# mathwrx/Decouple-and-Couple_Learning_in_Multi-Modal_Brain_Tumor_Segmentation

Hardware: AMD Instinct MI355X
Metric: training volumes/sec (4x128^3) (higher is better)
Workload: dtype bf16x3 forward (split-bf16 MFMA operands hi.hi+hi.lo+lo.hi: logits within 1e-3 of the fp32 reference) / bf16 data-gradient / bf16 weight-gradient MFMA operands; f32 accumulate, f32 storage, f32 master weights; 1 GPU; configs[1]: 1xMI355X, batch 2 per GPU, 4-modality 128^3 synthetic BraTS patches; fwd + softmax_dice + 4 sub-region/edge losses + bwd + Adam(amsgrad); random-init weights, dropout on; global_batch=2, parallelism=dp1, precision=bf16x3, dgrad_precision=bf16, wgrad_precision=bf16, mode=plan

## Files before the change

### decouple-and-couple_learning_in_multi-modal_brain_tumor_segmentation_amd/csrc/conv_args.h

```cpp
#pragma once
#include "common.h"

typedef __bf16 bf16x8 __attribute__((ext_vector_type(8)));
typedef unsigned u32x4 __attribute__((ext_vector_type(4)));

struct ConvArgsB {
  ConvGeom g;
  const float* x; const uint4* wpk; const float* bias; float* y;
  const float* in_scale; const float* in_shift; float in_slope;
  const float* residual; int r_ldc; const float* out_scale; double* stats;
  unsigned long long unused_[2];
  const float* nb_x; int nb_ldc; const float* nb_scale; const float* nb_shift; float nb_slope;
  int groups, x_goff, y_goff;
  const uint4* wpk_g[3]; const float* bias_g[3];
  const uint4* x16; const uint4* zero16;
  unsigned short* y16;
};

typedef __bf16 bf16x2_t __attribute__((ext_vector_type(2)));
typedef float f32x2_t __attribute__((ext_vector_type(2)));
__device__ __forceinline__ unsigned pack_bf16(float a, float b) {
  const f32x2_t f = {a, b};
  return __builtin_bit_cast(unsigned, __builtin_convertvector(f, bf16x2_t));
}
__device__ __forceinline__ float bf16_round(float a) { return (float)(__bf16)a; }
__device__ __forceinline__ void split_bf16(float a, float b, unsigned& hi, unsigned& lo) {
  hi = pack_bf16(a, b);
  const float ha = __builtin_bit_cast(float, hi << 16), hb = __builtin_bit_cast(float, hi & 0xffff0000u);
  lo = pack_bf16(a - ha, b - hb);
}
__device__ __forceinline__ float act01(float v, float slope) { return fmaxf(v, v * slope); }


static inline int cfg_extent(int op, int Di, int Hi, int Wi, int Do, int Ho, int Wo, int cd[3]) {
  cd[0] = Do; cd[1] = Ho; cd[2] = Wo;
  if (op == CWF_CONVT2) { cd[0] = Di; cd[1] = Hi; cd[2] = Wi; return 8; }
  if (op == CWF_CONV3_S2_DGRAD) { cd[0] = (Do + 1) / 2; cd[1] = (Ho + 1) / 2; cd[2] = (Wo + 1) / 2; return 8; }
  return 1;
}

int cwf_try_conv_ws(int op, int x3, ConvArgsB& a, hipStream_t st, int* rc);
int cwf_ws_takes_x16(int op, int N, int D, int H, int W, int Cin, int Cout);
int cwf_ws_takes_x3();
int cwf_try_conv_wsp(int op, int x3, int cfg_mt, int cfg_wm, ConvArgsB& a, hipStream_t st, int* rc);
int cwf_try_conv_wsd(int op, int x3, int cfg_mt, int cfg_wm, ConvArgsB& a, hipStream_t st, int* rc);

int conv_fp32_launch(const cwf_conv_args& d, hipStream_t st);
int conv_stem_launch(const cwf_conv_args& d, hipStream_t st);
int conv_s2c16_launch(const cwf_conv_args& d, hipStream_t st);
int wgrad_fp32_launch(const cwf_wgrad_args& d, int* nsplit_used, hipStream_t st);
```

### decouple-and-couple_learning_in_multi-modal_brain_tumor_segmentation_amd/csrc/conv_bf16.hip

```cpp
#include "common.h"
#include <cstdio>
#include <cstdlib>
#include <type_traits>

#include "conv_args.h"

#define CB_MAXS 13
struct StageSlots { int goff[CB_MAXS]; unsigned inb; int nslots; };

__device__ __forceinline__ void stage_slots_init(StageSlots& ss, const ConvGeom& g, int id0, int ih0, int iw0, int tid) {
  const int nvox_in = g.ID * g.IH * g.IW;
  ss.nslots = (nvox_in + 63) >> 6; ss.inb = 0u;
  const int dq = 64 / g.IW, dr = 64 - dq * g.IW;
  int iw = (tid >> 2) % g.IW, t2 = (tid >> 2) / g.IW;
  int ih = t2 % g.IH, idd = t2 / g.IH;
#pragma unroll
  for (int i = 0; i < CB_MAXS; ++i) {
    const int v = (tid >> 2) + 64 * i;
    const int gd = id0 + idd, gh = ih0 + ih, gw = iw0 + iw;
    const bool ok = v < nvox_in && gd >= 0 && gd < g.Di && gh >= 0 && gh < g.Hi && gw >= 0 && gw < g.Wi;
    ss.goff[i] = ok ? ((gd * g.Hi + gh) * g.Wi + gw) * g.x_ldc : 0;
    ss.inb |= ok ? (1u << i) : 0u;
    iw += dr; int adv = dq;
    if (iw >= g.IW) { iw -= g.IW; ++adv; }
// ... 1072 lines not shown
    const double reuse = 1.0 - 0.35 / (c.MT * c.NT) - 0.1 / MTOT;
    const double score = sp_eff * n_eff * fill * reuse;
    if (score > best_score) { best_score = score; best = c; }
  }
  return best;
}

template <int MT, int NT, int WM, bool X3>
int launch_cfg(const ConvArgsB& a, hipStream_t st) {
  constexpr int WN = 4 / WM;
  const ConvGeom& g = a.g;
  const size_t lds_tile = (size_t)g.ID * g.IH * g.IW * 16 * sizeof(unsigned short) * (X3 ? 2 : 1);
  const size_t lds_red = (size_t)4 * NT * 16 * 2 * sizeof(float);
  const size_t lds = lds_tile > lds_red ? lds_tile : lds_red;
  if (lds > 160 * 1024) return CWF_E_TOOLARGE;
  CWF_MAX_LDS_ONCE((&conv_bf16_kernel<MT, NT, WM, X3>));
  dim3 grid(g.tiles_d * g.tiles_h * g.tiles_w, cdiv(g.ntiles, WN * NT), g.N * g.ncls * (a.groups ? a.groups : 1));
  hipLaunchKernelGGL((conv_bf16_kernel<MT, NT, WM, X3>), grid, dim3(256), lds, st, a);
  CWF_LAUNCH_CHECK();
  return 0;
}
}

extern "C" int cwf_debug_conv_bf16_cfg(int op, int N, int Di, int Hi, int Wi, int Do, int Ho, int Wo, int Cout, int* mt_nt_wm) {
  if (!mt_nt_wm || N <= 0 || Di <= 0 || Hi <= 0 || Wi <= 0 || Do <= 0 || Ho <= 0 || Wo <= 0 || Cout <= 0 || op < CWF_CONV3_S1 ||
      op > CWF_CONVT2_DGRAD)
    return CWF_E_BADARG;
  int cd[3];
  const int ncls = cfg_extent(op, Di, Hi, Wi, Do, Ho, Wo, cd);
  const TileCfg c = choose_cfg(op, cd, ncls, N, cdiv(Cout, 16));
  mt_nt_wm[0] = c.MT; mt_nt_wm[1] = c.NT; mt_nt_wm[2] = c.WM;
  return 0;
}

static void c16_tap_order(ConvGeom& g) {
  int nat[27];
  for (int t = 0; t < 27; ++t) nat[t] = g.tapofs[t];
  for (int t = 0; t < 27; ++t) g.tapofs[t] = nat[c16_tap(t)];
}

static int conv_bf16_impl(const cwf_conv_args& d, hipStream_t st) {
  const int op = d.op, x3 = d.precision == CWF_BF16X3, N = d.N, Cin = d.Cin, Cout = d.Cout, y_ldc = d.y_ldc;
  const float* x = d.x16 ? reinterpret_cast<const float*>(d.x16) : d.x;
  const int x_ldc = d.x16 ? Cin : d.x_ldc;
  if (!x || !d.wpk || !d.y || N <= 0 || Cin <= 0 || Cout <= 0) return CWF_E_BADARG;
  if (d.nb_x && (!d.stats || !d.nb_scale || !d.nb_shift || d.nb_ldc < Cout)) return CWF_E_BADARG;
  if ((Cin & 3) || (x_ldc & 3) || x_ldc < Cin || y_ldc < Cout) return CWF_E_ALIGN;
  if (((uintptr_t)x & 15) || ((uintptr_t)d.wpk & 15)) return CWF_E_ALIGN;
  if (d.in_scale && !d.in_shift) return CWF_E_BADARG;
  ConvArgsB a;
  int cd[3];
  const int ncls = cfg_extent(op, d.Di, d.Hi, d.Wi, d.Do, d.Ho, d.Wo, cd);
  const TileCfg c = choose_cfg(op, cd, ncls, N, cdiv(Cout, 16));
  int rc = cwf_build_geom(a.g, op, N, d.Di, d.Hi, d.Wi, Cin, x_ldc, d.Do, d.Ho, d.Wo, Cout, y_ldc, c.MT * c.WM);
  if (rc) return rc;
  a.x = x; a.wpk = reinterpret_cast<const uint4*>(d.wpk); a.bias = d.bias; a.y = d.y; a.in_scale = d.in_scale; a.in_shift = d.in_shift;
  a.in_slope = d.x16 ? 1.f : d.in_slope; a.residual = d.residual; a.r_ldc = d.r_ldc; a.out_scale = d.out_scale; a.stats = d.stats;
  a.nb_x = d.nb_x; a.nb_ldc = d.nb_ldc; a.nb_scale = d.nb_scale; a.nb_shift = d.nb_shift; a.nb_slope = d.nb_x ? d.nb_slope : 1.f;
  a.groups = 0; a.x_goff = 0; a.y_goff = 0;
  a.x16 = reinterpret_cast<const uint4*>(d.x16); a.zero16 = reinterpret_cast<const uint4*>(d.zero16);
  a.y16 = reinterpret_cast<unsigned short*>(d.y16);
  for (int q = 0; q < 3; ++q) { a.wpk_g[q] = nullptr; a.bias_g[q] = nullptr; }
  if (d.x16 && Cin != 16) {
    int rcw = 0;
    return cwf_try_conv_ws(op, 0, a, st, &rcw) ? rcw : CWF_E_BADARG;
  }
  if (d.x16) {
    c16_tap_order(a.g);
    rc = cwf_build_geom(a.g, op, N, d.Di, d.Hi, d.Wi, Cin, x_ldc, d.Do, d.Ho, d.Wo, Cout, y_ldc, 16);
    if (rc) return rc;
    return launch_conv16s<false, true>(a, st);
  }
  {
    int ks, nt;
    if (pw_eligible(op, a, &ks, &nt)) {
      if (d.y16 && (op != CWF_CONV1 || (Cout & 3) || ((uintptr_t)d.y16 & 7))) return CWF_E_BADARG;
      return x3 ? dispatch_pw<true>(op, a, st, ks, nt) : dispatch_pw<false>(op, a, st, ks, nt);
    }
    if (d.y16) return CWF_E_BADARG;
  }
  {
    int rcw = 0;
    if (cwf_try_conv_wsp(op, x3, c.MT, c.WM, a, st, &rcw)) return rcw;
    if (cwf_try_conv_wsd(op, x3, c.MT, c.WM, a, st, &rcw)) return rcw;
    if (cwf_try_conv_ws(op, x3, a, st, &rcw)) return rcw;
  }
  if (op == CWF_CONV3_S1 && Cin <= 16 && Cout <= 16) c16_tap_order(a.g);
  if (op == CWF_CONV3_S1 && Cin <= 16 && Cout <= 16 && (int64_t)d.Do * d.Ho * d.Wo >= 32768) {
    rc = cwf_build_geom(a.g, op, N, d.Di, d.Hi, d.Wi, Cin, x_ldc, d.Do, d.Ho, d.Wo, Cout, y_ldc, 16);
    if (rc) return rc;
    return x3 ? launch_conv16s<true>(a, st) : launch_conv16s<false>(a, st);
  }
#define CWF_CFG(mt, nt, wm) if (c.MT == mt && c.NT == nt && c.WM == wm) return x3 ? launch_cfg<mt, nt, wm, true>(a, st) : launch_cfg<mt, nt, wm, false>(a, st);
  CWF_CFG(4, 4, 1) CWF_CFG(2, 4, 2) CWF_CFG(2, 4, 4) CWF_CFG(4, 2, 4) CWF_CFG(4, 1, 4)
  CWF_CFG(1, 4, 4) CWF_CFG(1, 2, 4) CWF_CFG(1, 2, 2) CWF_CFG(1, 1, 4)
#undef CWF_CFG
  return CWF_E_BADARG;
}

static int conv_grouped_impl(const cwf_conv_args& d, hipStream_t st) {
  const int op = d.op, x3 = d.precision == CWF_BF16X3, groups = d.groups, N = d.N, Cin = d.Cin, Cout = d.Cout;
  const int x_ldc = d.x_ldc, y_ldc = d.y_ldc, x_goff = d.x_goff, y_goff = d.y_goff;
  if (!d.x || !d.y || N <= 0 || Cin <= 0 || Cout <= 0) return CWF_E_BADARG;
  if ((Cin & 3) || (x_ldc & 3) || (x_goff & 3) || x_ldc < (groups - 1) * x_goff + Cin || y_ldc < (groups - 1) * y_goff + Cout) return CWF_E_ALIGN;
  if ((uintptr_t)d.x & 15) return CWF_E_ALIGN;
  ConvArgsB a;
  int cd[3];
  TileCfg c = choose_cfg(op, cd, cfg_extent(op, d.Di, d.Hi, d.Wi, d.Do, d.Ho, d.Wo, cd), N * groups, cdiv(Cout, 16));
  int rc = cwf_build_geom(a.g, op, N, d.Di, d.Hi, d.Wi, Cin, x_ldc, d.Do, d.Ho, d.Wo, Cout, y_ldc, c.MT * c.WM);
  if (rc) return rc;
  a.x = d.x; a.wpk = nullptr; a.bias = nullptr; a.y = d.y; a.in_scale = nullptr; a.in_shift = nullptr; a.in_slope = 1.f;
  a.residual = nullptr; a.r_ldc = 0; a.out_scale = nullptr; a.stats = nullptr;
  a.nb_x = nullptr; a.nb_ldc = 0; a.nb_scale = nullptr; a.nb_shift = nullptr; a.nb_slope = 1.f;
  a.groups = groups; a.x_goff = x_goff; a.y_goff = y_goff;
  a.x16 = nullptr; a.zero16 = nullptr; a.y16 = nullptr;
  for (int q = 0; q < 3; ++q) {
    a.wpk_g[q] = q < groups ? reinterpret_cast<const uint4*>(d.wpk_g[q]) : nullptr;
    a.bias_g[q] = q < groups ? d.bias_g[q] : nullptr;
    if (q < groups && (!d.wpk_g[q] || ((uintptr_t)d.wpk_g[q] & 15))) return CWF_E_ALIGN;
  }
  if (Cin <= 16 && Cout <= 16) c16_tap_order(a.g);
#define CWF_CFG(mt, nt, wm) if (c.MT == mt && c.NT == nt && c.WM == wm) return x3 ? launch_cfg<mt, nt, wm, true>(a, st) : launch_cfg<mt, nt, wm, false>(a, st);
  CWF_CFG(4, 4, 1) CWF_CFG(2, 4, 2) CWF_CFG(2, 4, 4) CWF_CFG(4, 2, 4) CWF_CFG(4, 1, 4)
  CWF_CFG(1, 4, 4) CWF_CFG(1, 2, 4) CWF_CFG(1, 2, 2) CWF_CFG(1, 1, 4)
#undef CWF_CFG
  return CWF_E_BADARG;
}

extern "C" int cwf_conv_x16_ok(int op, int N, int D, int H, int W, int Cin, int Cout) {
  if (op != CWF_CONV3_S1 || N <= 0 || D <= 0 || H <= 0 || W <= 0) return 0;
  if (Cin == 16 && Cout == 16) return (int64_t)D * H * W >= 32768 && (int64_t)N * D * H * W < (1ll << 30);
  return cwf_ws_takes_x16(op, N, D, H, W, Cin, Cout);
}

extern "C" int cwf_conv(const struct cwf_conv_args* args, void* stream) {
  if (!args) return CWF_E_BADARG;
  const cwf_conv_args& d = *args;
  if (d.precision != CWF_FP32 && d.precision != CWF_BF16X3 && d.precision != CWF_BF16) return CWF_E_BADARG;
  const bool fp32 = d.precision == CWF_FP32;
  hipStream_t st = cwf_stream(stream);
  if (d.groups) {
    if (d.groups < 2 || d.groups > 3 || d.op != CWF_CONV3_S1 || d.in_scale || d.residual || d.out_scale || d.stats || d.nb_x || d.x16 ||
        d.y16 || d.w_raw)
      return CWF_E_BADARG;
    if (!fp32) return conv_grouped_impl(d, st);
    for (int q = 0; q < d.groups; ++q) {
      cwf_conv_args g = d;
      g.groups = 0; g.x = d.x + q * d.x_goff; g.y = d.y + q * d.y_goff; g.wpk = d.wpk_g[q]; g.bias = d.bias_g[q];
      const int rc = conv_fp32_launch(g, st);
      if (rc) return rc;
    }
    return 0;
  }
  if (d.x16) {
    if (d.precision != CWF_BF16 || d.in_scale || d.out_scale || d.y16 || !d.zero16 || ((uintptr_t)d.x16 & 15) || ((uintptr_t)d.zero16 & 15))
      return CWF_E_BADARG;
    if (d.Do != d.Di || d.Ho != d.Hi || d.Wo != d.Wi || !cwf_conv_x16_ok(d.op, d.N, d.Di, d.Hi, d.Wi, d.Cin, d.Cout))
      return CWF_E_BADARG;
    return conv_bf16_impl(d, st);
  }
  if (d.y16) {
    if (d.nb_x || d.out_scale) return CWF_E_BADARG;
    if (!fp32 && d.op == CWF_CONV1) {
      const int rc = conv_bf16_impl(d, st);
      if (rc != CWF_E_BADARG) return rc;
    }
// ... 17 lines not shown
```

### decouple-and-couple_learning_in_multi-modal_brain_tumor_segmentation_amd/cwf/_lib.py

```python
from __future__ import annotations

import ctypes as C
import os

_HERE = os.path.dirname(os.path.abspath(__file__))
LIB_PATH = os.path.join(_HERE, "libcwf_hip.so")

P = C.c_void_p
I = C.c_int
L = C.c_int64
F = C.c_float
U = C.c_uint32
U64 = C.c_uint64
D = C.c_double

SIGNATURES = {
    "cwf_version": [],
    "cwf_conv": [P, P],
    "cwf_conv_x16_ok": [I, I, I, I, I, I, I],
    "cwf_debug_wsd": [I],
    "cwf_debug_wsd_launches": [],
    "cwf_wgrad": [P, P, P],
    "cwf_debug_wgrad_bf16_plan": [P, P],
    "cwf_debug_wgrad_bf16_name": [I],
    "cwf_debug_wgrad_s2": [I],
    "cwf_debug_wgrad_s2_launches": [],
    "cwf_gather_split_bf16": [P, I, L, P],
    "cwf_wgrad_nsplit": [I, I, I, I, I, I, I],
    "cwf_wgrad_partial_floats": [I, I, I, I, I, I, I],
    "cwf_wgrad_slab_floats": [I, I, I],
    "cwf_wgrad_reduce": [P, I, L, P, P, P, P],
    "cwf_gather_batched": [P, I, L, P],
    "cwf_in_finalize": [P, P, P, I, L, F, P],
    "cwf_in_stats": [P, I, P, I, L, I, P],
    "cwf_norm_act_add": [P, I, P, P, F, P, I, P, I, I, L, I, P],
    "cwf_in_bwd_stats": [P, I, P, I, P, P, F, P, I, L, I, P],
    "cwf_in_bwd_apply": [P, I, P, I, P, P, F, P, P, I, P, I, I, L, I, P],
    "cwf_in_bwd_apply_ex": [P, I, P, I, P, P, F, P, P, I, P, I, P, P, I, L, I, P],
    "cwf_norm_act_add_ex": [P, I, P, P, F, P, I, P, I, P, I, L, I, P],
    "cwf_to_bf16": [P, I, P, P, F, P, I, L, I, P],
    "cwf_gemm": [P, L, L, L, L, P, L, L, L, L, P, L, L, L, P, P, L, L, L, I, I, I, I, I, F, I, I, P],
    "cwf_layernorm_fwd": [P, P, P, P, P, P, I, I, F, P],
    "cwf_layernorm_bwd": [P, P, P, P, P, P, P, P, I, I, I, P],
    "cwf_softmax_rows": [P, L, I, I, P],
    "cwf_softmax_rows_bwd": [P, P, L, I, I, P],
    "cwf_gelu_bwd": [P, P, P, L, P],
    "cwf_colsum": [P, L, I, I, P, I, P],
    "cwf_window_to_tokens": [P, I, P, I, I, I, I, I, I, I, I, P],
    "cwf_tokens_to_window": [P, P, I, I, I, I, I, I, I, I, I, I, P],
    "cwf_token_scores": [P, P, L, P, I, I, I, P],
    "cwf_topk": [P, P, I, I, I, P],
    "cwf_gather_tokens": [P, P, P, L, P, F, P, I, I, I, I, P],
    "cwf_gather_tokens_bwd": [P, P, P, P, P, L, I, I, I, I, P],
    "cwf_scatter_rows": [P, P, P, L, L, P, L, P, I, I, I, I, P],
    "cwf_scatter_rows_bwd": [P, P, P, P, L, P, I, P, L, L, P, L, I, I, I, I, P],
    "cwf_upsample_softmax": [P, I, P, I, I, I, I, I, I, P],
    "cwf_upsample_softmax_bwd": [P, P, P, I, I, I, I, I, I, I, P, P],
    "cwf_channel_softmax": [P, I, P, L, I, P],
    "cwf_channel_softmax_bwd": [P, P, P, I, L, I, P],
    "cwf_dice_ce_sums": [P, P, U, P, I, L, I, P],
    "cwf_dice_ce_finalize": [P, P, P, I, L, I, P],
    "cwf_dice_ce_bwd": [P, P, U, P, P, P, I, L, I, P],
    "cwf_adam_amsgrad": [P, I, L, C.c_double, C.c_double, C.c_double, C.c_double, C.c_double, I, I, P, P],
    "cwf_adam_amsgrad_scaled": [P, I, L, C.c_double, C.c_double, C.c_double, C.c_double, C.c_double, I, I, P, F, P],
    "cwf_grad_add": [P, P, P, L, P],
    "cwf_grad_norm_clip": [P, L, F, F, P, P, P],
    "cwf_adam_amsgrad_ex": [P, I, L, C.c_double, C.c_double, C.c_double, C.c_double, C.c_double, I, I, P, F, P, P, F, P],
    "cwf_optim_step": [I, P, I, L, C.c_double, C.c_double, P, C.c_double, C.c_double, C.c_double, I, I, P, C.c_double, C.c_double, I, I,
                       F, P, P, F, P],
    "cwf_wgrad_reduce_batched": [P, I, P],
    "cwf_dropout_mask": [P, L, F, F, C.c_uint64, C.c_uint64, P],
    "cwf_mul": [P, P, P, L, P],
    "cwf_add": [P, P, P, L, P],
    "cwf_channel_scale": [P, I, P, P, I, I, L, I, P],
    "cwf_copy_strided": [P, I, P, I, L, I, P],
    "cwf_add3": [P, P, P, P, L, P],
    "cwf_bcast3": [P, P, L, P],
    "cwf_stats_channel_sum": [P, P, I, I, P],
    "cwf_gemm_ex": [P, P],
    "cwf_debug_gemm_panel": [I],
    "cwf_debug_gemm_panel_launches": [],
    "cwf_attn_fwd": [P, L, P, L, I, I, I, I, F, P, U64, F, P],
    "cwf_attn_bwd": [P, L, P, L, P, I, I, I, I, F, P, U64, F, P],
    "cwf_attn_bwd_ws": [P, L, P, L, P, I, I, I, I, F, P, U64, F, P, L, P],
    "cwf_attn_bwd_ws_bytes": [I, I, I],
    "cwf_debug_attn_split": [I],
    "cwf_debug_attn_split_waves": [I],
    "cwf_debug_attn_split_launches": [],
    "cwf_ln_pair_fwd": [P, P, I, P, P, P, P, P, P, P, I, I, F, P],
    "cwf_ln_pair_bwd": [P, P, P, P, P, I, P, P, P, P, P, P, P, P, P, I, I, I, P],
    "cwf_gelu_bwd_drop": [P, P, P, L, P, U64, F, P],
    "cwf_token_scores2": [P, P, L, P, L, P, P, I, I, I, P],
    "cwf_topk_inv": [P, P, P, P, P, P, I, I, I, P],
    "cwf_index_inv": [P, P, I, I, I, P],
    "cwf_gather_multi": [P, I, I, I, I, F, P, F, P],
    "cwf_scatter_inv": [P, P, P, L, L, P, L, P, P, I, I, I, P],
    "cwf_scatter_bwd": [P, P, P, P, P, P, L, L, P, L, P, L, P, L, L, P, L, I, I, I, I, P],
    "cwf_debug_scatter_bwd": [I],
    "cwf_token_grad": [P, P, P, L, P, P, P, L, P, L, P, U64, U64, F, P, I, I, I, I, P],
    "cwf_head_grad": [P, P, P, P, L, P, P, I, I, P],
    "cwf_dice_ce_finalize_multi": [P, P, P, P, I, I, L, I, P],
    "cwf_head_loss_sums": [P, I, I, P, P, P, I, I, I, I, I, P],
    "cwf_head_loss_bwd": [P, I, I, P, P, P, P, P, I, P, I, I, I, I, I, P],
    "cwf_head_loss_bwd_ex": [P, I, I, P, P, P, P, P, I, I, P, I, I, I, I, I, P],
# ... 114 lines not shown

class WgradArgs(C.Structure):
    _fields_ = [("op", I), ("precision", I),
                ("x", P), ("x_ldc", I), ("in_scale", P), ("in_shift", P), ("in_slope", F),
                ("dy", P), ("dy_ldc", I),
                ("dy_scale", P), ("xa16", P), ("dy16", P), ("zero16", P),
                ("partial", P),
                ("groups", I), ("x_g", P * 3), ("dy_g", P * 3), ("partial_g", P * 3),
                ("N", I), ("Di", I), ("Hi", I), ("Wi", I), ("Cin", I), ("Do", I), ("Ho", I), ("Wo", I), ("Cout", I)]


PRECISION = {"fp32": 0, "bf16x3": 1, "bf16": 2}


class LnGroupParams(C.Structure):
    _fields_ = [(n, P * 4) for n in ("g1", "b1", "g2", "b2", "dg1", "db1", "dg2", "db2")]


class GatherJob(C.Structure):
    _fields_ = [("feats", P), ("index", P), ("head", P), ("out", P), ("head_bstride", L), ("out_bstride", L), ("T", I),
                ("drop_off", C.c_uint64), ("head_g", P * 4), ("group_B", I)]


class PrepSample(C.Structure):
    _fields_ = [("image", P), ("label", P), ("S0", I), ("S1", I), ("S2", I), ("o0", I), ("o1", I), ("o2", I), ("flip", I),
                ("intensity", I), ("scale", F * 4), ("shift", F * 4)]


class PrepAffineSample(C.Structure):
    _fields_ = PrepSample._fields_ + [("m", F * 9)]


class PrepElasticSample(C.Structure):
    _fields_ = PrepAffineSample._fields_ + [("disp", P), ("G0", I), ("G1", I), ("G2", I)]


class IntensitySample(C.Structure):
    _fields_ = [("taps", (F * 7) * 4), ("amp", F * 4), ("key", U64), ("gamma", F * 4), ("blur", I), ("noise", I), ("gam", I)]


class FocalParams(C.Structure):
    _fields_ = [("fn", D), ("fp", D), ("exponent", D), ("smooth", D), ("gamma", D), ("ce_ratio", D), ("class_weight", D * 4)]


INTENSITY_TILE = (10, 10, 32)


def intensity_ws_floats(nb, crop):
    tiles = 1
    for c, t in zip(crop, INTENSITY_TILE):
        tiles *= (int(c) + t - 1) // t
    return 8 * int(nb) * tiles


class AcquireSample(C.Structure):
    _fields_ = [("bias", P * 4), ("G0", I), ("G1", I), ("G2", I), ("bias_mask", I), ("contrast_mask", I), ("lowres_mask", I),
                ("factor", F * 4), ("lattice", (I * 3) * 4)]


ACQUIRE_TILE = (32, 8, 32)


def acquire_ws_doubles(nb, crop):
    tiles = 1
    for c, t in zip(crop, ACQUIRE_TILE):
        tiles *= (int(c) + t - 1) // t
    return 12 * int(nb) * tiles


WINDOW_MAX_STARTS = 128


class WindowGrid(C.Structure):
    _fields_ = [("B", I), ("S", I * 3), ("r", I * 3), ("n", I * 3), ("start", (I * WINDOW_MAX_STARTS) * 3)]


class WindowBox(C.Structure):
    _fields_ = [("full", I * 3), ("lo", I * 3)]


NORM_WS_DOUBLES = 2568
GRADNORM_WS_DOUBLES = 1024
RULE_ADAMW, RULE_SGD = 1, 2
RESTYPE_INT64 = {"cwf_debug_wsd_launches", "cwf_debug_wgrad_s2_launches", "cwf_debug_gemm_panel_launches", "cwf_debug_attn_split_launches", "cwf_attn_bwd_ws_bytes", "cwf_wgrad_partial_floats", "cwf_wgrad_slab_floats", "cwf_hausdorff_workspace", "cwf_components_workspace",
                 "cwf_lesionwise_workspace", "cwf_surface_metrics_workspace", "cwf_lesionwise_ex_workspace", "cwf_signed_distance_workspace",
                 "cwf_topk_ce_workspace", "cwf_focal_workspace", "cwf_lovasz_workspace", "cwf_class_locations_workspace", "cwf_nonzero_box_workspace"}
LOCATIONS_TILE = 16384
NONZERO_BOX_TILE = 4096

_lib = None


class CwfError(RuntimeError):
    pass


def load():
    global _lib
    if _lib is not None:
        return _lib
    if not os.path.exists(LIB_PATH):
        raise CwfError("libcwf_hip.so is not built (%s); run `python __graft_entry__.py` or `make -C csrc`. "
                       "There is no CPU fallback." % LIB_PATH)
    lib = C.CDLL(LIB_PATH)
    for name, args in SIGNATURES.items():
        fn = getattr(lib, name)
        fn.argtypes = args
        fn.restype = L if name in RESTYPE_INT64 else I
    lib.cwf_arch.restype = C.c_char_p
    lib.cwf_arch.argtypes = []
    lib.cwf_plan_last_error.restype = C.c_char_p
    lib.cwf_plan_last_error.argtypes = []
    lib.cwf_debug_wgrad_bf16_name.restype = C.c_char_p
    _lib = lib
    return lib


def check(rc, name):
    if rc != 0:
        raise CwfError("%s failed with status %d" % (name, rc))
```

### include/cwf_hip.h

```cpp
#ifndef CWF_HIP_H
#define CWF_HIP_H
#include <stdint.h>
#ifdef __cplusplus
extern "C" {
#endif

#define CWF_E_BADARG   (-1)
#define CWF_E_TOOLARGE (-2)
#define CWF_E_ALIGN    (-3)

int cwf_version(void);
const char* cwf_arch(void);

enum { CWF_CONV3_S1 = 0, CWF_CONV3_S2 = 1, CWF_CONV1 = 2, CWF_CONVT2 = 3, CWF_CONV3_S2_DGRAD = 4, CWF_CONVT2_DGRAD = 5 };
enum { CWF_FP32 = 0, CWF_BF16X3 = 1, CWF_BF16 = 2 };

struct cwf_conv_args {
  int op, precision;
  const float* x; int x_ldc; const void* wpk; const float* bias; float* y; int y_ldc;
  const float* in_scale; const float* in_shift; float in_slope;
  const float* residual; int r_ldc; const float* out_scale; double* stats;
  const float* nb_x; int nb_ldc; const float* nb_scale; const float* nb_shift; float nb_slope;
  const void* x16; const void* zero16; void* y16;
  const float* w_raw;
  int groups, x_goff, y_goff; const void* wpk_g[3]; const float* bias_g[3];
  int N, Di, Hi, Wi, Cin, Do, Ho, Wo, Cout;
};
int cwf_conv(const struct cwf_conv_args* args , void* stream);
int cwf_conv_x16_ok(int op, int N, int D, int H, int W, int Cin, int Cout);
int cwf_debug_wsd(int v);
long long cwf_debug_wsd_launches(void);

int cwf_wgrad_nsplit(int op, int N, int Do, int Ho, int Wo, int Cin, int Cout);
int64_t cwf_wgrad_partial_floats(int op, int N, int Do, int Ho, int Wo, int Cin, int Cout);
int64_t cwf_wgrad_slab_floats(int op, int Cin, int Cout);
struct cwf_wgrad_args {
  int op, precision;
  const float* x; int x_ldc; const float* in_scale; const float* in_shift; float in_slope;
  const float* dy; int dy_ldc;
  const float* dy_scale; const void* xa16; const void* dy16; const void* zero16;
  float* partial;
  int groups; const float* x_g[3]; const float* dy_g[3]; float* partial_g[3];
  int N, Di, Hi, Wi, Cin, Do, Ho, Wo, Cout;
};
int cwf_wgrad(const struct cwf_wgrad_args* args , int* nsplit_used , void* stream);
enum cwf_wgrad_bf16_instance {
  CWF_WGB_WGRAD16 = 0, CWF_WGB_WGRAD16_X3,
  CWF_WGB_PW_1_1_1, CWF_WGB_PW_2_1_1, CWF_WGB_PW_4_2_1, CWF_WGB_PW_8_4_1,
  CWF_WGB_PW_1_1_8, CWF_WGB_PW_2_2_8,
  CWF_WGB_S1_1, CWF_WGB_S1_2,
  CWF_WGB_TILED_7_1, CWF_WGB_TILED_7_1_X3, CWF_WGB_TILED_7_2, CWF_WGB_TILED_7_2_X3,
  CWF_WGB_TILED_2_1, CWF_WGB_TILED_2_1_X3, CWF_WGB_TILED_2_2, CWF_WGB_TILED_2_2_X3,
  CWF_WGB_TILED_2_4, CWF_WGB_TILED_2_4_X3,
  CWF_WGB_WGRAD16D, CWF_WGB_S1D,
  CWF_WGB_COUNT
};
enum { CWF_WGB_WALK_RANGES = 0, CWF_WGB_WALK_STRIDED = 1, CWF_WGB_WALK_PW = 2 };
#define CWF_WGB_PLAN_FIELDS 15
int cwf_debug_wgrad_bf16_plan(const struct cwf_wgrad_args* args , int64_t* out );
const char* cwf_debug_wgrad_bf16_name(int instance);
int cwf_debug_wgrad_s2(int v);
long long cwf_debug_wgrad_s2_launches(void);
int cwf_wgrad_reduce(const float* partial, int nsplit, int64_t slab_floats,
                     const int32_t* inv_map, float* dW, float* db, void* stream);
struct cwf_wgrad_reduce_desc { const float* partial; const int32_t* inv; float* dW; float* db; int64_t slab; int32_t nsplit; int32_t pad_; };
int cwf_wgrad_reduce_batched(const struct cwf_wgrad_reduce_desc* table, int nlayers, void* stream);

struct cwf_gather_desc { const float* src; float* dst; const int32_t* map; int64_t n; };

int cwf_gather_split_bf16(const struct cwf_gather_desc* table, int nlayers, int64_t max_n, void* stream);

int cwf_gather_batched(const struct cwf_gather_desc* table, int nlayers, int64_t max_n, void* stream);

int cwf_in_finalize(const double* stats, float* scale, float* shift, int NC, int64_t V, float eps, void* stream);
int cwf_in_stats(const float* x, int x_ldc, double* stats, int N, int64_t V, int C, void* stream);
int cwf_norm_act_add(const float* x, int x_ldc, const float* scale, const float* shift, float slope,
                     const float* residual, int r_ldc, float* y, int y_ldc, int N, int64_t V, int C, void* stream);
int cwf_in_bwd_stats(const float* dy, int dy_ldc, const float* x, int x_ldc, const float* scale, const float* shift,
                     float slope, double* sums, int N, int64_t V, int C, void* stream);
int cwf_in_bwd_apply(const float* dy, int dy_ldc, const float* x, int x_ldc, const float* scale, const float* shift,
                     float slope, const double* sums, const float* dx_add, int a_ldc, float* dx, int dx_ldc,
                     int N, int64_t V, int C, void* stream);

int cwf_in_bwd_apply_ex(const float* dy, int dy_ldc, const float* x, int x_ldc, const float* scale, const float* shift,
                        float slope, const double* sums, const float* dx_add, int a_ldc, float* dx, int dx_ldc,
                        void* dx16, void* xa16, int N, int64_t V, int C, void* stream);
int cwf_norm_act_add_ex(const float* x, int x_ldc, const float* scale, const float* shift, float slope,
                        const float* residual, int r_ldc, float* y, int y_ldc, void* y16, int N, int64_t V, int C, void* stream);
int cwf_to_bf16(const float* x, int x_ldc, const float* scale, const float* shift, float slope, void* y16,
                int N, int64_t V, int C, void* stream);
int cwf_gemm(const float* A, int64_t sa_m, int64_t sa_k, int64_t sa_zb, int64_t sa_zh,
             const float* B, int64_t sb_k, int64_t sb_n, int64_t sb_zb, int64_t sb_zh,
             float* C, int64_t sc_m, int64_t sc_zb, int64_t sc_zh,
             const float* bias, const float* residual, int64_t sr_m, int64_t sr_zb, int64_t sr_zh,
             int M, int Nn, int K, int ZB, int ZH, float alpha, int act, int accumulate, void* stream);
struct cwf_gemm_args {
  const float* A; int64_t sa_m, sa_k, sa_zb, sa_zh;
  const float* B; int64_t sb_k, sb_n, sb_zb, sb_zh;
  float* C; int64_t sc_m, sc_zb, sc_zh;
  const float* bias; const float* residual; int64_t sr_m, sr_zb, sr_zh;
  int M, N, K, ZB, ZH; float alpha; int act; int accumulate;
  const float* A2; int split_n;
  const float* B2; int split_m;
  float* C2;
  float* rowsum; int rowsum_acc;
  const uint64_t* rng;
  uint64_t a_drop_off, a_drop_n; float a_drop_p, a_drop_p2;
  uint64_t c_drop_off, c_drop_n; float c_drop_p, c_drop_p2;
  const float* B_tab[4]; const float* bias_tab[4]; float* C_tab[4]; float* rowsum_tab[4];
};
int cwf_gemm_ex(const struct cwf_gemm_args* args , void* stream);
int cwf_debug_gemm_panel(int v);
long long cwf_debug_gemm_panel_launches(void);

// ... 321 lines not shown
```

Measured before the change: 124.4 volumes/s.

## Add warp-specialized stride-2 conv kernel with producer/consumer LDS pipeline

Adds a new kernel for stride-2 3x3x3 convolutions. Four producer waves load fp32 input, split it to bf16 hi/lo and write a phase-deinterleaved halo tile into double-buffered LDS. Four consumer waves hold the weights in registers and run the MFMA loop over 27 taps paired into 14 k-steps, with a persistent per-slot tile schedule and an XCD-aware block permutation. By default it is routed only to three specific encoder shapes, replacing the generic wsd/ws paths for those shapes. In exchange it adds a large specialized kernel with a high register footprint and shape-specific routing.

```diff
diff --git a/decouple-and-couple_learning_in_multi-modal_brain_tumor_segmentation_amd/csrc/conv_args.h b/decouple-and-couple_learning_in_multi-modal_brain_tumor_segmentation_amd/csrc/conv_args.h
--- a/decouple-and-couple_learning_in_multi-modal_brain_tumor_segmentation_amd/csrc/conv_args.h
+++ b/decouple-and-couple_learning_in_multi-modal_brain_tumor_segmentation_amd/csrc/conv_args.h
@@ -44,6 +44,7 @@
 int cwf_ws_takes_x3();
 int cwf_try_conv_wsp(int op, int x3, int cfg_mt, int cfg_wm, ConvArgsB& a, hipStream_t st, int* rc);
 int cwf_try_conv_wsd(int op, int x3, int cfg_mt, int cfg_wm, ConvArgsB& a, hipStream_t st, int* rc);
+int cwf_try_conv_s2w(int op, int x3, int cfg_mt, ConvArgsB& a, hipStream_t st, int* rc);
 
 int conv_fp32_launch(const cwf_conv_args& d, hipStream_t st);
 int conv_stem_launch(const cwf_conv_args& d, hipStream_t st);
diff --git a/decouple-and-couple_learning_in_multi-modal_brain_tumor_segmentation_amd/csrc/conv_bf16.hip b/decouple-and-couple_learning_in_multi-modal_brain_tumor_segmentation_amd/csrc/conv_bf16.hip
--- a/decouple-and-couple_learning_in_multi-modal_brain_tumor_segmentation_amd/csrc/conv_bf16.hip
+++ b/decouple-and-couple_learning_in_multi-modal_brain_tumor_segmentation_amd/csrc/conv_bf16.hip
@@ -1178,6 +1178,7 @@
   {
     int rcw = 0;
     if (cwf_try_conv_wsp(op, x3, c.MT, c.WM, a, st, &rcw)) return rcw;
+    if (cwf_try_conv_s2w(op, x3, c.MT, a, st, &rcw)) return rcw;
     if (cwf_try_conv_wsd(op, x3, c.MT, c.WM, a, st, &rcw)) return rcw;
     if (cwf_try_conv_ws(op, x3, a, st, &rcw)) return rcw;
   }
diff --git a/decouple-and-couple_learning_in_multi-modal_brain_tumor_segmentation_amd/csrc/conv_s2w.hip b/decouple-and-couple_learning_in_multi-modal_brain_tumor_segmentation_amd/csrc/conv_s2w.hip
--- /dev/null
+++ b/decouple-and-couple_learning_in_multi-modal_brain_tumor_segmentation_amd/csrc/conv_s2w.hip
@@ -0,0 +1,310 @@
+#include "conv_args.h"
+#include <cstdlib>
+#include <type_traits>
+
+#define S2W_ROW 34
+#define S2W_NVOX (5 * 5 * 33)
+#define S2W_SLOTS 13
+#define S2W_IMG (5 * 5 * S2W_ROW * 32)
+
+struct S2wWork { int ngroups, slots, tiles, xcd_perm, tiles_d, tiles_h, tiles_w; };
+
+__host__ __device__ constexpr int s2w_tap_bytes(int t) {
+  return (((t / 9) * 5 + (t / 3) % 3) * S2W_ROW + ((t % 3) & 1) * 17 + ((t % 3) >> 1)) * 32;
+}
+
+template <int M, int T, bool X3>
+__global__ __launch_bounds__(512) void conv_s2w_kernel(const ConvArgsB a, const S2wWork wk) {
+  constexpr int WN = M;
+  constexpr int IMGS = X3 ? 2 : 1;
+  constexpr int A_BUF = IMGS * S2W_IMG;
+  extern __shared__ float4 lds4[];
+  char* const A0 = reinterpret_cast<char*>(lds4);
+  const ConvGeom& g = a.g;
+  const int nch = g.nchunks;
+  const int tid = threadIdx.x, lane = tid & 63;
+  const int wave = __builtin_amdgcn_readfirstlane(tid >> 6);
+
+  int cgrp, slot;
+  {
+    const int b = blockIdx.x;
+    if (wk.xcd_perm) {
+      const int per = gridDim.x >> 3, j = b >> 3;
+      cgrp = j % wk.ngroups;
+      slot = (b & 7) * (per / wk.ngroups) + j / wk.ngroups;
+    } else {
+      cgrp = b % wk.ngroups;
+      slot = b / wk.ngroups;
+    }
+  }
+  const int t_begin = (int)(((int64_t)slot * wk.tiles) / wk.slots), t_end = (int)(((int64_t)(slot + 1) * wk.tiles) / wk.slots);
+  const int ntw = t_end - t_begin;
+  const int tiles_per_n = wk.tiles_d * wk.tiles_h * wk.tiles_w;
+
+  if (wave < 4) {
+    const int mh = wave / WN, jt = cgrp * WN + wave % WN;
+    const int r = lane & 15, kq = lane >> 4;
+    const bool second = (kq >> 1) != 0;
+    const int a_lane = r * 32 + (kq & 1) * 16 + (M == 2 ? mh * (2 * 5 * S2W_ROW * 32) : 0);
+    auto row_bytes = [](int m) { return M == 4 ? ((2 * (m >> 1)) * 5 + 2 * (m & 1)) * S2W_ROW * 32 : (2 * m) * S2W_ROW * 32; };
+
+    f32x4 acc[T][M];
+#pragma unroll
+    for (int k = 0; k < T; ++k)
+#pragma unroll
+      for (int m = 0; m < M; ++m) acc[k][m] = (f32x4){0.f, 0.f, 0.f, 0.f};
+    float s1 = 0.f, s2 = 0.f;
+    double d1 = 0.0, d2 = 0.0;
+    int stats_n = -1;
+    const int co = jt * 16 + r;
+    const float bv = a.bias ? a.bias[co] : 0.f;
+    auto fold_stats = [&]() {
+      float u1 = s1, u2 = s2;
+      u1 += __shfl_xor(u1, 16, 64); u1 += __shfl_xor(u1, 32, 64);
+      u2 += __shfl_xor(u2, 16, 64); u2 += __shfl_xor(u2, 32, 64);
+      d1 += (double)u1; d2 += (double)u2;
+      s1 = 0.f; s2 = 0.f;
+    };
+    auto flush_stats = [&]() {
+      if (kq == 0) {
+        atomic_add_f64(a.stats + ((int64_t)stats_n * g.Cout + co) * 2 + 0, d1);
+        atomic_add_f64(a.stats + ((int64_t)stats_n * g.Cout + co) * 2 + 1, d2);
+      }
+      d1 = 0.0; d2 = 0.0;
+    };
+
+    u32x4 bh[14], bl[14];
+    const char* wsrc = reinterpret_cast<const char*>(a.wpk + ((int64_t)g.cls_wbase16[0] + jt) * 128);
+    auto load_b = [&](int chunk) {
+      unsigned lo_ = (unsigned)lane * 32u;
+      asm volatile("" : "+v"(lo_));
+#pragma unroll
+      for (int s = 0; s < 14; ++s) {
+        const char* p = wsrc + (int64_t)(chunk * 14 + s) * g.ntiles * 2048;
+        bh[s] = *reinterpret_cast<const u32x4*>(p + lo_);
+        if (X3) bl[s] = *reinterpret_cast<const u32x4*>(p + lo_ + 16);
+      }
+    };
+
+    auto mfma_item = [&](int buf, auto KK) {
+      constexpr int k = decltype(KK)::value;
+      const char* ah0 = A0 + buf * A_BUF + a_lane;
+      int sec = second;
+      asm volatile("" : "+v"(sec));
+      u32x4 fa[2][M], fl[M];
+      auto tap_of = [&](int s) {
+        const int c0 = s2w_tap_bytes(2 * s), c1 = s2w_tap_bytes(2 * s + 1 < 27 ? 2 * s + 1 : 2 * s);
+        return sec ? c1 : c0;
+      };
+      auto rd_hi = [&](int s, int p) {
+        const int to = tap_of(s);
+#pragma unroll
+        for (int m = 0; m < M; ++m) fa[p][m] = *reinterpret_cast<const u32x4*>(ah0 + row_bytes(m) + to);
+      };
+      auto rd_lo = [&](int s) {
+        const int to = tap_of(s);
+#pragma unroll
+        for (int m = 0; m < M; ++m) fl[m] = *reinterpret_cast<const u32x4*>(ah0 + S2W_IMG + row_bytes(m) + to);
+      };
+      rd_hi(0, 0);
+#pragma unroll
+      for (int s = 0; s < 14; ++s) {
+        const int p = s & 1;
+        if (X3) rd_lo(s);
+        if (s + 1 < 14) rd_hi(s + 1, p ^ 1);
+#pragma unroll
+        for (int m = 0; m < M; ++m)
+          acc[k][m] = __builtin_amdgcn_mfma_f32_16x16x32_bf16(__builtin_bit_cast(bf16x8, fa[p][m]), __builtin_bit_cast(bf16x8, bh[s]), acc[k][m], 0, 0, 0);
+        if (X3) {
+#pragma unroll
+          for (int m = 0; m < M; ++m)
+            acc[k][m] = __builtin_amdgcn_mfma_f32_16x16x32_bf16(__builtin_bit_cast(bf16x8, fa[p][m]), __builtin_bit_cast(bf16x8, bl[s]), acc[k][m], 0, 0, 0);
+#pragma unroll
+          for (int m = 0; m < M; ++m)
+            acc[k][m] = __builtin_amdgcn_mfma_f32_16x16x32_bf16(__builtin_bit_cast(bf16x8, fl[m]), __builtin_bit_cast(bf16x8, bh[s]), acc[k][m], 0, 0, 0);
+        }
+        __builtin_amdgcn_sched_barrier(0);
+      }
+    };
+
+    auto epilogue = [&](int tile, auto KK) {
+      constexpr int k = decltype(KK)::value;
+      asm volatile("" : "+s"(tile));
+      const int n = tile / tiles_per_n;
+      int bx = tile - n * tiles_per_n;
+      const int tw = bx % wk.tiles_w; bx /= wk.tiles_w;
+      const int th_ = bx % wk.tiles_h, td_ = bx / wk.tiles_h;
+      if (a.stats && n != stats_n) {
+        if (stats_n >= 0) flush_stats();
+        stats_n = n;
+      }
+      const int ow0 = tw * 16;
+      unsigned yo[4];
+#pragma unroll
+      for (int i = 0; i < 4; ++i) { yo[i] = (unsigned)((kq * 4 + i) * g.y_ldc + co) * 4u; asm volatile("" : "+v"(yo[i])); }
+#pragma unroll
+      for (int m = 0; m < M; ++m) {
+        const int od = td_ * 2 + (M == 4 ? (m >> 1) : mh), oh = th_ * 2 + (M == 4 ? (m & 1) : m);
+        if (od < g.Do && oh < g.Ho) {
+          char* yb = reinterpret_cast<char*>(a.y + ((((int64_t)n * g.Do + od) * g.Ho + oh) * g.Wo + ow0) * g.y_ldc);
+#pragma unroll
+          for (int i = 0; i < 4; ++i) {
+            if (ow0 + kq * 4 + i < g.Wo) {
+              const float v = acc[k][m][i] + bv;
+              *reinterpret_cast<float*>(yb + yo[i]) = v;
+              s1 += v; s2 = fmaf(v, v, s2);
+            }
+          }
+          if (a.stats) fold_stats();
+          else { s1 = 0.f; s2 = 0.f; }
+        }
+        acc[k][m] = (f32x4){0.f, 0.f, 0.f, 0.f};
+      }
+    };
+
+    int i = 0;
+    for (int t0 = 0; t0 < ntw; t0 += T) {
+      const int nk = min(T, ntw - t0);
+      for (int c = 0; c < nch; ++c) {
+        load_b(c);
+        auto item = [&](auto KK) {
+          asm volatile("s_waitcnt lgkmcnt(0)\n\ts_barrier" ::: "memory");
+          mfma_item(i & 1, KK);
+          if (c == nch - 1) epilogue(t_begin + t0 + decltype(KK)::value, KK);
+          ++i;
+        };
+        item(std::integral_constant<int, 0>{});
+        if (T > 1 && nk > 1) item(std::integral_constant<int, (T > 1 ? 1 : 0)>{});
+        if (T > 2 && nk > 2) item(std::integral_constant<int, (T > 2 ? 2 : 0)>{});
+        if (T > 3 && nk > 3) item(std::integral_constant<int, (T > 3 ? 3 : 0)>{});
+      }
+    }
+    if (a.stats && stats_n >= 0) flush_stats();
+  } else {
+    const int lt = tid - 256;
+    const int q = lt & 3;
+    const int ni = ntw * nch;
+    struct Item { int tile, chunk; };
+    auto item_of = [&](int it) {
+      const int per_round = T * nch;
+      const int rd = it / per_round, w = it - rd * per_round;
+      const int nk = min(T, ntw - rd * T);
+      const int c = w / nk, k = w - c * nk;
+      Item o; o.tile = t_begin + rd * T + k; o.chunk = c;
+      return o;
+    };
+    int hv[S2W_SLOTS]; unsigned lofs[S2W_SLOTS];
+#pragma unroll
+    for (int i = 0; i < S2W_SLOTS; ++i) {
+      const int v = min((lt >> 2) + 64 * i, S2W_NVOX - 1);
+      const int iw = v % 33, t2 = v / 33, ih = t2 % 5, idd = t2 / 5;
+      hv[i] = idd | (ih << 4) | (iw << 8);
+      lofs[i] = (unsigned)((((idd * 5 + ih) * S2W_ROW) + (iw & 1) * 17 + (iw >> 1)) * 32 + q * 8);
+    }
+    const bool last_slot = (lt >> 2) + 64 * (S2W_SLOTS - 1) < S2W_NVOX;
+    const unsigned ldc4 = (unsigned)g.x_ldc * 4u;
+    f32x4 pf[S2W_SLOTS];
+    unsigned pf_inb = 0u;
+    auto fetch = [&](int it) {
+      const Item itm = item_of(it);
+      const int n = itm.tile / tiles_per_n;
+      int bx = itm.tile - n * tiles_per_n;
+      const int tw = bx % wk.tiles_w; bx /= wk.tiles_w;
+      const int th_ = bx % wk.tiles_h, td_ = bx / wk.tiles_h;
+      const int d0 = td_ * 4 - 1, h0 = th_ * 4 - 1, w0 = tw * 32 - 1;
+      const char* xb = reinterpret_cast<const char*>(a.x + (int64_t)n * g.Di * g.Hi * g.Wi * g.x_ldc + itm.chunk * 16);
+      unsigned inb = 0u;
+#pragma unroll
+      for (int i = 0; i < S2W_SLOTS; ++i) {
+        const int gd = d0 + (hv[i] & 15), gh = h0 + ((hv[i] >> 4) & 15), gw = w0 + (hv[i] >> 8);
+        const bool ok = (i < S2W_SLOTS - 1 || last_slot) & ((unsigned)gd < (unsigned)g.Di) & ((unsigned)gh < (unsigned)g.Hi) & ((unsigned)gw < (unsigned)g.Wi);
+        const unsigned lin = (unsigned)((gd * g.Hi + gh) * g.Wi + gw) * ldc4 + (unsigned)q * 16u;
+        const unsigned boff = ok ? lin : (unsigned)q * 16u;
+        pf[i] = *reinterpret_cast<const f32x4*>(xb + boff);
+        inb |= ok ? (1u << i) : 0u;
+      }
+      pf_inb = inb;
+    };
+    auto convert = [&](int buf) {
+      char* xh = A0 + buf * A_BUF;
+      const unsigned inb = pf_inb;
+#pragma unroll
+      for (int i = 0; i < S2W_SLOTS; ++i) {
+        if (i == S2W_SLOTS - 1 && !last_slot) continue;
+        uint2 h, l;
+        if (X3) { split_bf16(pf[i][0], pf[i][1], h.x, l.x); split_bf16(pf[i][2], pf[i][3], h.y, l.y); }
+        else { h.x = pack_bf16(pf[i][0], pf[i][1]); h.y = pack_bf16(pf[i][2], pf[i][3]); l = make_uint2(0u, 0u); }
+        const bool was = (inb >> i) & 1u;
+        h.x = was ? h.x : 0u; h.y = was ? h.y : 0u; l.x = was ? l.x : 0u; l.y = was ? l.y : 0u;
+        *reinterpret_cast<uint2*>(xh + lofs[i]) = h;
+        if (X3) *reinterpret_cast<uint2*>(xh + S2W_IMG + lofs[i]) = l;
+      }
+    };
+    if (ni > 0) { fetch(0); convert(0); }
+    if (ni > 1) fetch(1);
+    for (int it = 0; it < ni; ++it) {
+      asm volatile("s_waitcnt lgkmcnt(0)\n\ts_barrier" ::: "memory");
+      if (it + 1 < ni) {
+        convert((it + 1) & 1);
+        if (it + 2 < ni) fetch(it + 2);
+      }
+    }
+  }
+}
+
+namespace {
+template <int M, int T, bool X3>
+int launch_s2w(const ConvArgsB& a, const S2wWork& wk, int grid, hipStream_t st) {
+  const size_t lds = (size_t)2 * (X3 ? 2 : 1) * S2W_IMG;
+  CWF_MAX_LDS_ONCE((&conv_s2w_kernel<M, T, X3>));
+  hipLaunchKernelGGL((conv_s2w_kernel<M, T, X3>), dim3(grid), dim3(512), lds, st, a, wk);
+  CWF_LAUNCH_CHECK();
+  return 0;
+}
+template <int M, int T>
+int launch_s2w_x(int x3, const ConvArgsB& a, const S2wWork& wk, int grid, hipStream_t st) {
+  return x3 ? launch_s2w<M, T, true>(a, wk, grid, st) : launch_s2w<M, T, false>(a, wk, grid, st);
+}
+}
+
+static int g_s2w = 1;
+extern "C" int cwf_debug_s2w(int v) { const int old = g_s2w; g_s2w = v; return old; }
+static long long g_s2w_launches = 0;
+extern "C" long long cwf_debug_s2w_launches() { return g_s2w_launches; }
+
+static bool s2w_routed(int Cin, int Cout, int Do, int Ho, int Wo) {
+  static const int cls[][5] = {{32, 64, 32, 32, 32}, {32, 32, 32, 32, 32}, {64, 128, 16, 16, 16}};
+  for (const auto& c : cls)
+    if (Cin == c[0] && Cout == c[1] && Do == c[2] && Ho == c[3] && Wo == c[4]) return true;
+  return false;
+}
+
+int cwf_try_conv_s2w(int op, int x3, int cfg_mt, ConvArgsB& a, hipStream_t st, int* rc) {
+  const ConvGeom& g = a.g;
+  if (!g_s2w || op != CWF_CONV3_S2) return 0;
+  if (a.groups || a.out_scale || a.nb_x || a.residual || a.in_scale || a.in_slope != 1.f || a.x16 || a.y16) return 0;
+  if (g.Cin < 32 || (g.Cin & 15) || !(g.Cout == 32 || (g.Cout & 63) == 0)) return 0;
+  if (g.x_ldc < g.Cin || (g.x_ldc & 3) || g.y_ldc < g.Cout) return 0;
+  if (g.Do != (g.Di + 1) / 2 || g.Ho != (g.Hi + 1) / 2 || g.Wo != (g.Wi + 1) / 2) return 0;
+  if ((int64_t)g.Di * g.Hi * g.Wi * g.x_ldc * 4 >= (1ll << 31)) return 0;
+  if (a.stats && cfg_mt != 1) return 0;
+  if (g_s2w == 1 && !s2w_routed(g.Cin, g.Cout, g.Do, g.Ho, g.Wo)) return 0;
+  S2wWork wk;
+  const int m = g.Cout == 32 ? 2 : 4;
+  wk.ngroups = g.Cout / (16 * m);
+  if (wk.ngroups > 32) return 0;
+  wk.tiles_d = cdiv(g.Do, 2); wk.tiles_h = cdiv(g.Ho, 2); wk.tiles_w = cdiv(g.Wo, 16);
+  const int64_t tiles = (int64_t)g.N * wk.tiles_d * wk.tiles_h * wk.tiles_w;
+  if (tiles >= (1ll << 30)) return 0;
+  wk.tiles = (int)tiles;
+  const int per = (32 / wk.ngroups) * wk.ngroups;
+  wk.slots = 8 * (per / wk.ngroups);
+  wk.xcd_perm = 1;
+  if (wk.slots > wk.tiles) { wk.slots = wk.tiles; wk.xcd_perm = 0; }
+  const int grid = wk.slots * wk.ngroups;
+  const int per_wg = (wk.tiles + wk.slots - 1) / wk.slots;
+  if (m == 4) *rc = per_wg > 1 ? launch_s2w_x<4, 4>(x3, a, wk, grid, st) : launch_s2w_x<4, 1>(x3, a, wk, grid, st);
+  else *rc = per_wg > 1 ? launch_s2w_x<2, 4>(x3, a, wk, grid, st) : launch_s2w_x<2, 1>(x3, a, wk, grid, st);
+  if (*rc == 0) ++g_s2w_launches;
+  return 1;
+}
diff --git a/decouple-and-couple_learning_in_multi-modal_brain_tumor_segmentation_amd/cwf/_lib.py b/decouple-and-couple_learning_in_multi-modal_brain_tumor_segmentation_amd/cwf/_lib.py
--- a/decouple-and-couple_learning_in_multi-modal_brain_tumor_segmentation_amd/cwf/_lib.py
+++ b/decouple-and-couple_learning_in_multi-modal_brain_tumor_segmentation_amd/cwf/_lib.py
@@ -20,6 +20,8 @@
     "cwf_conv_x16_ok": [I, I, I, I, I, I, I],
     "cwf_debug_wsd": [I],
     "cwf_debug_wsd_launches": [],
+    "cwf_debug_s2w": [I],
+    "cwf_debug_s2w_launches": [],
     "cwf_wgrad": [P, P, P],
     "cwf_debug_wgrad_bf16_plan": [P, P],
     "cwf_debug_wgrad_bf16_name": [I],
@@ -300,7 +302,7 @@
 NORM_WS_DOUBLES = 2568
 GRADNORM_WS_DOUBLES = 1024
 RULE_ADAMW, RULE_SGD = 1, 2
-RESTYPE_INT64 = {"cwf_debug_wsd_launches", "cwf_debug_wgrad_s2_launches", "cwf_debug_gemm_panel_launches", "cwf_debug_attn_split_launches", "cwf_attn_bwd_ws_bytes", "cwf_wgrad_partial_floats", "cwf_wgrad_slab_floats", "cwf_hausdorff_workspace", "cwf_components_workspace",
+RESTYPE_INT64 = {"cwf_debug_wsd_launches", "cwf_debug_s2w_launches", "cwf_debug_wgrad_s2_launches", "cwf_debug_gemm_panel_launches", "cwf_debug_attn_split_launches", "cwf_attn_bwd_ws_bytes", "cwf_wgrad_partial_floats", "cwf_wgrad_slab_floats", "cwf_hausdorff_workspace", "cwf_components_workspace",
                  "cwf_lesionwise_workspace", "cwf_surface_metrics_workspace", "cwf_lesionwise_ex_workspace", "cwf_signed_distance_workspace",
                  "cwf_topk_ce_workspace", "cwf_focal_workspace", "cwf_lovasz_workspace", "cwf_class_locations_workspace", "cwf_nonzero_box_workspace"}
 LOCATIONS_TILE = 16384
diff --git a/include/cwf_hip.h b/include/cwf_hip.h
--- a/include/cwf_hip.h
+++ b/include/cwf_hip.h
@@ -30,6 +30,8 @@
 int cwf_conv_x16_ok(int op, int N, int D, int H, int W, int Cin, int Cout);
 int cwf_debug_wsd(int v);
 long long cwf_debug_wsd_launches(void);
+int cwf_debug_s2w(int v);
+long long cwf_debug_s2w_launches(void);
 
 int cwf_wgrad_nsplit(int op, int N, int Do, int Ho, int Wo, int Cin, int Cout);
 int64_t cwf_wgrad_partial_floats(int op, int N, int Do, int Ho, int Wo, int Cin, int Cout);
```

Result: no change. 125.0 volumes/s, median of 6 (+0.5%).
